# jc-bao/gym-formation

Hardware: AMD Instinct MI355X
Metric: env-steps/sec (higher is better)
Workload: dtype f32

## Files before the change

### gym-formation_amd/csrc/fg_obs_writers.hpp

```cpp
#ifndef FG_OBS_WRITERS_HPP_
#define FG_OBS_WRITERS_HPP_

#include "fg_common.hpp"

namespace fg {

template <class V2> FG_DEV V2 lds_if(bool c, const V2* __restrict__ p, int idx_if_true) {
    V2 t = p[c ? idx_if_true : 0];
    t.x = c ? t.x : 0.0f; t.y = c ? t.y : 0.0f;
    return t;
}

constexpr bool FG_ROWS_MERGED = true;
template <int NC, int NW, int E, int PACE = 0>
FG_DEV void write_obs_rows(const real2* __restrict__ tables0, int env_stride, int w,
                           real2* __restrict__ out_env0, size_t env_units, int El, int parts,
                           int wg_part = 0, int wg_parts = 1, bool pace_on = true) {
    constexpr int N = NC;
    constexpr int WPE = (E >= NW) ? 1 : NW / E;
    constexpr int ESTEP = (E >= NW) ? NW : 1;
    static_assert((E >= NW) ? (E % NW == 0) : (NW % E == 0), "waves and envs must tile");
    const int lane = threadIdx.x & 63;
    const int row0 = (E >= NW) ? 0 : w % WPE;
    constexpr unsigned ROWU = 3u * N;
    for (int ee = (E >= NW) ? w : w / WPE; ee < El; ee += (E >= NW ? ESTEP : E)) {
        const real2* __restrict__ AA = tables0 + (size_t)ee * env_stride;
        real2* __restrict__ out = out_env0 + (size_t)ee * env_units;
        if constexpr (N <= 64) {
            constexpr int RW = 64 / N;
            const int rsub = lane / N, u = lane - rsub * N;
            const bool act = rsub < RW;
            const real2 zero = make_real2(0.f, 0.f);
            const real2 Pm = lds_if(act && u >= 1, AA, u - 1);
            const real2 Pu = lds_if(act && u >= 1, AA, u);
            const int xoff = (u == 0) ? 4 * N : 0;
            constexpr int CS = (2 * N + 63) / 64;
            constexpr int RS = (2 * N <= 64) ? 64 / (2 * N) : 1;
            const int ssub = (2 * N <= 64) ? lane / (2 * N) : 0;
            const int sidx = (2 * N <= 64) ? lane - ssub * 2 * N : lane;
            real2 sv[CS];
#pragma unroll
            for (int c = 0; c < CS; ++c)
                sv[c] = lds_if(ssub < RS && sidx + 64 * c < 2 * N, AA, N + sidx + 64 * c);
#pragma unroll 2
            for (int rb = row0; rb < N; rb += RW * WPE) {
                const int r = rb + rsub * WPE;
                if ((parts & 1) && act && r < N) {
                    const real2 x = AA[xoff + r];
                    const real2 c = (u - 1 >= r) ? Pu : Pm;
                    out[(unsigned)r * ROWU + (unsigned)u] = make_real2(c.x - x.x, c.y - x.y);
                }
#pragma unroll
                for (int k0 = 0; k0 < RW; k0 += RS) {
                    const int rs = rb + (k0 + ssub) * WPE;
                    if ((parts & 2) && ssub < RS && k0 + ssub < RW && rs < N) {
#pragma unroll
                        for (int c = 0; c < CS; ++c)
                            if (sidx + 64 * c < 2 * N) out[(unsigned)rs * ROWU + (unsigned)(N + sidx + 64 * c)] = sv[c];
                    }
                }
            }
        } else if constexpr (FG_ROWS_MERGED && ((3 * N + 63) / 64 < (N + 63) / 64 + (2 * N + 63) / 64)) {
            constexpr int CR = (3 * N + 63) / 64;
            constexpr int C_MIX = N / 64;
            real2 Pm[CR], Pu[CR];
#pragma unroll
            for (int c = 0; c < CR; ++c) {
                const int u = lane + 64 * c;
                if (c <= C_MIX) {
                    const bool dyn = u >= 1 && u < N, stat = u >= N && u < 3 * N;
                    Pm[c] = lds_if(dyn || stat, AA, stat ? u : u - 1);
                    Pu[c] = lds_if(dyn || stat, AA, u);
                } else {
                    Pm[c] = Pu[c] = lds_if(u < 3 * N, AA, u);
                }
            }
            const int nshare = WPE * wg_parts, share = wg_part * WPE + row0;
            const int PER = (N + nshare - 1) / nshare;
            const int r_end = min(N, (share + 1) * PER);
#pragma unroll 2
            for (int r = share * PER; r < r_end; ++r) {
                const real2 xp = AA[r];
                const real2 x0 = AA[(lane == 0 ? 4 * N : 0) + r];
                real2* __restrict__ orow = out + (unsigned)r * ROWU;
#pragma unroll
                for (int c = 0; c < CR; ++c) {
                    const int u = lane + 64 * c;
                    real2 val;
                    if (c < C_MIX || (c == C_MIX && (N % 64) == 0)) {
                        const real2 x = (c == 0) ? x0 : xp;
                        const real2 cc = (u - 1 >= r) ? Pu[c] : Pm[c];
                        val = make_real2(cc.x - x.x, cc.y - x.y);
                    } else if (c == C_MIX) {
                        const bool dyn = u < N;
                        const real2 x = (c == 0) ? x0 : xp;
                        const real2 cc = (u - 1 >= r) ? Pu[c] : Pm[c];
                        val = make_real2(cc.x - (dyn ? x.x : 0.0f), cc.y - (dyn ? x.y : 0.0f));
                    } else {
                        val = Pu[c];
                    }
                    if (u < 3 * N) orow[u] = val;
                }
                if (PACE > 0 && pace_on) __builtin_amdgcn_s_sleep(PACE);
            }
        } else {
            constexpr int CD = (N + 63) / 64, CS = (2 * N + 63) / 64;
            const real2 zero = make_real2(0.f, 0.f);
            real2 Pm[CD], Pu[CD], sv[CS];
#pragma unroll
            for (int c = 0; c < CD; ++c) {
                const int u = lane + 64 * c;
                Pm[c] = lds_if(u >= 1 && u < N, AA, u - 1);
                Pu[c] = lds_if(u >= 1 && u < N, AA, u);
            }
#pragma unroll
            for (int c = 0; c < CS; ++c) sv[c] = lds_if(lane + 64 * c < 2 * N, AA, N + lane + 64 * c);
            const int nshare = WPE * wg_parts, share = wg_part * WPE + row0;
            const int PER = (N + nshare - 1) / nshare;
            const int r_end = min(N, (share + 1) * PER);
#pragma unroll 2
            for (int r = share * PER; r < r_end; ++r) {
                const real2 xp = AA[r];
                const real2 x0 = AA[(lane == 0 ? 4 * N : 0) + r];
                real2* __restrict__ orow = out + (unsigned)r * ROWU;
#pragma unroll
                for (int c = 0; c < CD; ++c) {
                    const int u = lane + 64 * c;
                    const real2 x = (c == 0) ? x0 : xp;
                    const real2 cc = (u - 1 >= r) ? Pu[c] : Pm[c];
                    if ((parts & 1) && u < N) orow[u] = make_real2(cc.x - x.x, cc.y - x.y);
                }
#pragma unroll
                for (int c = 0; c < CS; ++c)
                    if ((parts & 2) && lane + 64 * c < 2 * N) orow[N + lane + 64 * c] = sv[c];
                if (PACE > 0 && pace_on) __builtin_amdgcn_s_sleep(PACE);
            }
        }
    }
}

template <int NC, int RT> constexpr int tile_units() { return (3 * NC * RT + 16 + 2 + 1) & ~1; }

template <int NC, int NW, int E, int RT, bool STREAM>
FG_DEV void write_obs_tiled(const float2* __restrict__ tables0, int env_stride, int w, float2* __restrict__ tiles,
                            float2* __restrict__ out_env0, size_t unit0, size_t env_units, int El) {
    constexpr int N = NC;
    constexpr int WPE = (E >= NW) ? 1 : NW / E;
    static_assert((E >= NW) ? (E % NW == 0) : (NW % E == 0), "waves and envs must tile");
    static_assert(N <= 32 && N % RT == 0, "tiled writer: N <= 32, RT divides N");
    constexpr unsigned ROWU = 3u * N, TU = ROWU * RT;
    constexpr int TILES_ENV = N / RT;
    constexpr int MY_TILES = (TILES_ENV + WPE - 1) / WPE;
    const int lane = threadIdx.x & 63;
    float2* tile0 = tiles + w * 2 * tile_units<NC, RT>();
    constexpr int RW = 64 / N;
    const int rsub = lane / N, u = lane - rsub * N;
    const bool act = rsub < RW;
    const int xoff = (u == 0) ? 4 * N : 0;
    constexpr int RS = 64 / (2 * N);
    const int ssub = lane / (2 * N), sidx = lane - ssub * 2 * N;
    const int e_first = (E >= NW) ? w : w / WPE, e_step = (E >= NW) ? NW : E;
    const int t_first = (E >= NW) ? 0 : w % WPE;
    const int n_env = (El > e_first) ? (El - e_first + e_step - 1) / e_step : 0;
    const int total = n_env * MY_TILES;

    constexpr unsigned ENVU = ROWU * N;
    const unsigned pad = (unsigned)(env_units - ENVU);
    static_assert(!STREAM || (E >= NW && NC >= 16), "streaming form: waves own whole envs, rows of >= 16 units");
    const bool own = STREAM && ((unit0 & 15) == 0) && (pad == 0 || (pad < 16 && (env_units & 15) == 0));
    auto head_units = [&](int ee) -> unsigned {
        return (own && pad == 0) ? (16u - (unsigned)(((size_t)ee * env_units) & 15)) & 15u : 0u;
    };
    auto extra_units = [&](int ee) -> unsigned {
        if (!own) return 0u;
        if (pad) return pad;
        return (ee + 1 < El) ? head_units(ee + 1) : 0u;
    };

    int cur_env = -1;
    const float2* __restrict__ AA = tables0;
    float2 Pm = make_float2(0.f, 0.f), Pu = Pm, sv = Pm;
    auto locate = [&](int t, int& ee, int& r0) {
        const int ie = t / MY_TILES, it = t - ie * MY_TILES;
        ee = e_first + ie * e_step;
        r0 = (t_first + it * WPE) * RT;
    };
    auto compose = [&](int t) {
        int ee, r0; locate(t, ee, r0);
        if (r0 >= N) return;
        if (ee != cur_env) {
            cur_env = ee;
            AA = tables0 + (size_t)ee * env_stride;
            Pm = lds_if(act && u >= 1, AA, u - 1);
            Pu = lds_if(act && u >= 1, AA, u);
            sv = lds_if(ssub < RS, AA, N + sidx);
        }
        const unsigned par = (unsigned)((unit0 + (size_t)ee * env_units + (size_t)r0 * ROWU) & 1);
        float2* img = tile0 + (t & 1) * tile_units<NC, RT>() + par;
#pragma unroll
        for (int rb = 0; rb < RT; rb += RW) {
            const int rl = rb + rsub;
            if (act && rl < RT) {
                const int r = r0 + rl;
                const float2 x = AA[xoff + r];
                const float2 c = (u - 1 >= r) ? Pu : Pm;
                img[(unsigned)rl * ROWU + (unsigned)u] = make_float2(c.x - x.x, c.y - x.y);
            }
        }
#pragma unroll
        for (int rb = 0; rb < RT; rb += RS) {
            const int rl = rb + ssub;
            if (ssub < RS && rl < RT) img[(unsigned)rl * ROWU + (unsigned)(N + sidx)] = sv;
        }
        if (STREAM && r0 + RT == N) {
            const unsigned x = extra_units(ee);
            if ((unsigned)lane < x) {
                float2 val = make_float2(0.f, 0.f);
                if (pad == 0) {
                    static_assert(ROWU >= 16, "the line remainder must stay inside row 0 of the next env");
                    const float2* __restrict__ A1 = tables0 + (size_t)(ee + 1) * env_stride;
                    const float2 a = A1[lane == 0 ? 3 * N : lane], b = A1[0];
                    const bool rel = lane >= 1 && lane < N;
                    val = make_float2(a.x - (rel ? b.x : 0.f), a.y - (rel ? b.y : 0.f));
                }
                img[TU + (unsigned)lane] = val;
            }
        }
    };
    auto stream = [&](int t) {
        int ee, r0; locate(t, ee, r0);
        if (r0 >= N) return;
        const unsigned par = (unsigned)((unit0 + (size_t)ee * env_units + (size_t)r0 * ROWU) & 1);
        const float2* img = tile0 + (t & 1) * tile_units<NC, RT>() + par;
        float2* __restrict__ out = out_env0 + (size_t)ee * env_units + (size_t)r0 * ROWU;
        if constexpr (!STREAM) {
            if (par && lane == 0) out[0] = img[0];
            constexpr unsigned NPMAX = TU >> 1;
            const unsigned npair = (TU - par) >> 1;
            const f32x4* src4 = reinterpret_cast<const f32x4*>(img + par);
            f32x4* __restrict__ dst4 = reinterpret_cast<f32x4*>(out + par);
#pragma unroll
            for (unsigned q0 = 0; q0 < NPMAX; q0 += 64) {
                const unsigned q = q0 + lane;
                if (q < npair) dst4[q] = src4[q];
            }
            if (((TU - par) & 1u) && lane == 63) out[TU - 1] = img[TU - 1];
        } else {
            const unsigned s = (r0 == 0) ? head_units(ee) : 0u;
            const unsigned end = TU + ((r0 + RT == N) ? extra_units(ee) : 0u);
            const unsigned p2 = (par + s) & 1u;
            if (p2 && lane == 0) out[s] = img[s];
            constexpr unsigned NPMAX = (TU + 16) >> 1;
            const unsigned npair = (end - s - p2) >> 1;
            const f32x4* src4 = reinterpret_cast<const f32x4*>(img + s + p2);
            f32x4* __restrict__ dst4 = reinterpret_cast<f32x4*>(out + s + p2);
            constexpr unsigned NFULL = ((TU - 16) >> 1) / 64;
#pragma unroll
            for (unsigned c = 0; c < NFULL; ++c) {
                const f32x4 v = src4[c * 64 + lane];
                asm volatile("s_waitcnt lgkmcnt(0)" ::: "memory");
                dst4[c * 64 + lane] = v;
                asm volatile("" ::: "memory");
                __builtin_amdgcn_s_sleep(1);
            }
#pragma unroll
            for (unsigned q0 = NFULL * 64; q0 < NPMAX; q0 += 64) {
                const unsigned q = q0 + lane;
                if (q < npair) dst4[q] = src4[q];
            }
            if (((end - s - p2) & 1u) && lane == 63) out[end - 1] = img[end - 1];
        }
    };
    if (total > 0) compose(0);
    for (int t = 0; t < total; ++t) {
        if (t + 1 < total) compose(t + 1);
        stream(t);
    }
}

constexpr int FG_WR_GATHER = 64;
template <int NC> constexpr int gather_passes() { return (3 * NC * NC / 2 + 2 + 63) / 64; }
template <int NC> constexpr int gather_lut_units() { return 2 * gather_passes<NC>() * 64 * 2; }

template <int NC>
FG_DEV void build_gather_lut(uint4* __restrict__ lut, int t, int nthreads) {
    constexpr int N = NC, ROWU = 3 * N, TU = ROWU * N, P = gather_passes<NC>() * 64;
    static_assert(N >= 2 && 5 * N < 65536, "gather writer: table offsets are 16-bit, the table's zeros are the 0 operand");
    auto operands = [&](int unit, unsigned& a, unsigned& b) {
        const int r = unit / ROWU, u = unit - r * ROWU;
        if (u == 0) { a = N; b = 4 * N + r; }
        else if (u < N) { a = (u - 1 >= r) ? u : u - 1; b = r; }
        else { a = u; b = N; }
    };
    for (int e = t; e < 2 * P; e += nthreads) {
        const int par = e / P, q = e - par * P;
        const int npair = (TU - par) >> 1;
        const bool tail = ((TU - par) & 1) != 0;
        int unit = -1, kind = 0;
        if (q < npair) { unit = 2 * q + par; kind = 2; }
        else if (par && q == npair) { unit = 0; kind = 1; }
        else if (tail && q == npair + par) { unit = TU - 1; kind = 1; }
        unsigned a0 = N, b0 = N, a1 = N, b1 = N;
        if (kind >= 1) operands(unit, a0, b0);
        if (kind == 2) operands(unit + 1, a1, b1);
        lut[e] = make_uint4(a0 | (b0 << 16), a1 | (b1 << 16), (unsigned)(unit < 0 ? 0 : unit) | ((unsigned)kind << 16), 0u);
    }
}

template <int NC> struct GatherEntries {
    uint32_t ab0[gather_passes<NC>()], ab1[gather_passes<NC>()], dst[gather_passes<NC>()];
    int phase = -1;
};

template <int NC, int NW, int E>
FG_DEV void write_obs_gather(const float2* __restrict__ tables0, int env_stride, int w, const uint4* __restrict__ lut,
                             float2* __restrict__ out_env0, size_t unit0, size_t env_units, int El, GatherEntries<NC>& cache) {
    constexpr int PASSES = gather_passes<NC>(), P = PASSES * 64;
    const int lane = threadIdx.x & 63;
    for (int ee = w; ee < El; ee += NW) {
        const float2* __restrict__ T = tables0 + (size_t)ee * env_stride;
        const size_t first = unit0 + (size_t)ee * env_units;
        float2* __restrict__ out = out_env0 + (size_t)ee * env_units;
        const int phase = (int)(first & 1);
        if (phase != cache.phase) {
            const uint4* __restrict__ L = lut + phase * P + lane;
#pragma unroll
            for (int c = 0; c < PASSES; ++c) {
                const uint4 t = L[c * 64];
                cache.ab0[c] = t.x; cache.ab1[c] = t.y; cache.dst[c] = t.z;
            }
            cache.phase = phase;
        }
        f32x4 val[PASSES];
#pragma unroll
        for (int c = 0; c < PASSES; ++c) {
            const float2 A0 = T[cache.ab0[c] & 0xffffu], B0 = T[cache.ab0[c] >> 16], A1 = T[cache.ab1[c] & 0xffffu], B1 = T[cache.ab1[c] >> 16];
            val[c] = (f32x4){A0.x - B0.x, A0.y - B0.y, A1.x - B1.x, A1.y - B1.y};
        }
#pragma unroll
        for (int c = 0; c < PASSES; ++c) {
            const unsigned kind = cache.dst[c] >> 16, dst = cache.dst[c] & 0xffffu;
            if (kind == 2) *reinterpret_cast<f32x4*>(out + dst) = val[c];
            else if (kind == 1) out[dst] = make_float2(val[c].x, val[c].y);
        }
    }
}

template <int NC, int NW, int E, int CHMAX = 4> struct SpanGather {
    static constexpr int ENVU = 3 * NC * NC, PIECES = E * ENVU / 2, INSTR = (PIECES + 63) / 64, MINE = (INSTR + NW - 1) / NW;
    static_assert((E * ENVU) % 2 == 0, "an even number of units per workgroup span");
    static FG_DEV void setup(uint2* __restrict__ lut, int w, int env_stride) {
        const int lane = threadIdx.x & 63;
        auto operands = [&](int unit) -> uint32_t {
            const int e = unit / ENVU, q = unit - e * ENVU;
            const int r = q / (3 * NC), u = q - r * (3 * NC);
            uint32_t a, b;
            if (u == 0) { a = NC; b = 4 * NC + r; }
            else if (u < NC) { a = (u - 1 >= r) ? u : u - 1; b = r; }
            else { a = u; b = NC; }
            const uint32_t base = (uint32_t)(e * env_stride);
            return (a + base) | ((b + base) << 16);
        };
        for (int t = 0; t < MINE; ++t) {
            const int piece = (w + NW * t) * 64 + lane;
            if (piece < PIECES) lut[piece] = make_uint2(operands(2 * piece), operands(2 * piece + 1));
        }
    }
    static FG_DEV void write(const uint2* __restrict__ lut, const float2* __restrict__ tables0, int w, float2* __restrict__ out) {
        const int lane = threadIdx.x & 63;
        f32x4* const out4 = reinterpret_cast<f32x4*>(out);
        constexpr int CH = MINE < CHMAX ? MINE : CHMAX;
#pragma unroll
        for (int t0 = 0; t0 < MINE; t0 += CH) {
            uint2 ent[CH];
#pragma unroll
            for (int c = 0; c < CH; ++c) {
                const int piece = (w + NW * (t0 + c)) * 64 + lane;
                ent[c] = lut[(t0 + c < MINE && piece < PIECES) ? piece : 0];
            }
            f32x4 val[CH];
#pragma unroll
            for (int c = 0; c < CH; ++c) {
                const float2 A0 = tables0[ent[c].x & 0xffffu], B0 = tables0[ent[c].x >> 16];
                const float2 A1 = tables0[ent[c].y & 0xffffu], B1 = tables0[ent[c].y >> 16];
                val[c] = (f32x4){A0.x - B0.x, A0.y - B0.y, A1.x - B1.x, A1.y - B1.y};
            }
#pragma unroll
            for (int c = 0; c < CH; ++c) {
                const int piece = (w + NW * (t0 + c)) * 64 + lane;
                if (t0 + c < MINE && piece < PIECES) out4[piece] = val[c];
            }
        }
    }
};

constexpr int FG_WR_OBS_F16 = 65, FG_WR_OBS_BF16 = 66;
constexpr bool roll_writer_obs16(int wr) { return wr == FG_WR_OBS_F16 || wr == FG_WR_OBS_BF16; }
template <int NC> constexpr int obs16_rows() { return NC > 9 ? 9 : NC; }
template <int NC, int NW, int E> constexpr int obs16_envs() { return NC <= 9 ? E / NW : 1; }
template <int NC, int NW, int E> constexpr int obs16_tile_words() { return (obs16_envs<NC, NW, E>() * obs16_rows<NC>() * 3 * NC + 3 + 3) & ~3; }

#if !FG_F64
typedef uint32_t u32x4 __attribute__((ext_vector_type(4)));
template <int FMT> FG_DEV uint32_t obs16_pack(float x, float y) {
    if constexpr (FMT == FG_WR_OBS_F16) {
        typedef _Float16 h2 __attribute__((ext_vector_type(2)));
        const h2 v = {(_Float16)x, (_Float16)y};
        return __builtin_bit_cast(uint32_t, v);
    } else {
        typedef __bf16 b2 __attribute__((ext_vector_type(2)));
        const b2 v = {(__bf16)x, (__bf16)y};
        return __builtin_bit_cast(uint32_t, v);
    }
}

template <int NC, int NW, int E, int FMT>
FG_DEV void write_obs16(const float2* __restrict__ tables0, int env_stride, int w, uint32_t* __restrict__ tiles,
                        uint32_t* __restrict__ span, size_t unit0, int El) {
    constexpr int N = NC, RT = obs16_rows<NC>(), ET = obs16_envs<NC, NW, E>(), WORDS = obs16_tile_words<NC, NW, E>();
    static_assert(N <= 32 && N % RT == 0 && E >= NW && E % NW == 0, "16-bit writer: N <= 32, whole rows per tile, whole envs per wave");
    static_assert(ET == 1 || RT == N, "a tile of several envs holds them whole");
    constexpr unsigned ROWU = 3u * N, ENVU = ROWU * N, TU = ROWU * RT;
    constexpr int TILES_ENV = N / RT;
    const int lane = threadIdx.x & 63;
    uint32_t* const tile0 = tiles + w * 2 * WORDS;
    constexpr int RW = 64 / N;
    const int rsub = lane / N, u = lane - rsub * N;
    const bool act = rsub < RW;
    const int xoff = (u == 0) ? 4 * N : 0;
    constexpr int RS = 64 / (2 * N);
    const int ssub = lane / (2 * N), sidx = lane - ssub * 2 * N;
    const int n_env = (El > w) ? (El - w + NW - 1) / NW : 0;
    const int total = ET == 1 ? n_env * TILES_ENV : (w * ET < El ? 1 : 0);
    auto locate = [&](int t, int& ee, int& r0, int& ne) {
        if constexpr (ET == 1) {
            const int ie = t / TILES_ENV;
            ee = w + ie * NW; r0 = (t - ie * TILES_ENV) * RT; ne = 1;
        } else {
            ee = w * ET; r0 = 0; ne = min(ET, El - ee);
        }
    };
    auto compose = [&](int t) {
        int ee, r0, ne; locate(t, ee, r0, ne);
        const unsigned par = (unsigned)((unit0 + (size_t)ee * ENVU + (size_t)r0 * ROWU) & 3);
        uint32_t* img = tile0 + (t & 1) * WORDS + par;
        for (int j = 0; j < ne; ++j, img += TU) {
            const float2* __restrict__ AA = tables0 + (size_t)(ee + j) * env_stride;
            const float2 Pm = lds_if(act && u >= 1, AA, u - 1);
            const float2 Pu = lds_if(act && u >= 1, AA, u);
            const float2 sv = lds_if(ssub < RS, AA, N + sidx);
#pragma unroll
            for (int rb = 0; rb < RT; rb += RW) {
                const int rl = rb + rsub;
                if (act && rl < RT) {
                    const int r = r0 + rl;
                    const float2 x = AA[xoff + r];
                    const float2 c = (u - 1 >= r) ? Pu : Pm;
                    img[(unsigned)rl * ROWU + (unsigned)u] = obs16_pack<FMT>(c.x - x.x, c.y - x.y);
                }
            }
            const uint32_t svp = obs16_pack<FMT>(sv.x, sv.y);
#pragma unroll
            for (int rb = 0; rb < RT; rb += RS) {
                const int rl = rb + ssub;
                if (ssub < RS && rl < RT) img[(unsigned)rl * ROWU + (unsigned)(N + sidx)] = svp;
            }
        }
    };
    auto stream = [&](int t) {
        int ee, r0, ne; locate(t, ee, r0, ne);
        const size_t first = (size_t)ee * ENVU + (size_t)r0 * ROWU;
        const unsigned par = (unsigned)((unit0 + first) & 3);
        const uint32_t* img = tile0 + (t & 1) * WORDS + par;
        uint32_t* __restrict__ out = span + first;
        const unsigned n = (unsigned)ne * TU;
        const unsigned head = (4u - par) & 3u;
        if ((unsigned)lane < head) out[lane] = img[lane];
        const unsigned nq = (n - head) >> 2;
        const u32x4* src4 = reinterpret_cast<const u32x4*>(img + head);
        u32x4* __restrict__ dst4 = reinterpret_cast<u32x4*>(out + head);
        constexpr unsigned NQMAX = ((unsigned)ET * TU) >> 2;
#pragma unroll
        for (unsigned q0 = 0; q0 < NQMAX; q0 += 64) {
            const unsigned q = q0 + lane;
            if (q < nq) dst4[q] = src4[q];
        }
        const unsigned tail = (n - head) & 3u, t0 = head + 4u * nq;
        if ((unsigned)lane < tail) out[t0 + lane] = img[t0 + lane];
    };
    if (total > 0) compose(0);
    for (int t = 0; t < total; ++t) {
        if (t + 1 < total) compose(t + 1);
        stream(t);
    }
}
#endif

}

#endif
```

Baseline: 341.3 million.

## Add compile-time scheduled streaming observation writer interleaving tile build and drain

Adds a specialized observation writer for 27 agents with 9-row tiles and two envs per wave. It unrolls the tile schedule at compile time and interleaves building the next LDS tile with draining the current one through 16-byte global stores. The goal is to hide LDS latency behind global stores and keep output writes aligned. In exchange it adds a lot of geometry-specific code, plus manual waitcnt and sleep instructions that may not suit other configurations.

```diff
diff --git a/gym-formation_amd/csrc/fg_obs_writers.hpp b/gym-formation_amd/csrc/fg_obs_writers.hpp
--- a/gym-formation_amd/csrc/fg_obs_writers.hpp
+++ b/gym-formation_amd/csrc/fg_obs_writers.hpp
@@ -1,6 +1,8 @@
 #ifndef FG_OBS_WRITERS_HPP_
 #define FG_OBS_WRITERS_HPP_
 
+#include <type_traits>
+#include <utility>
 #include "fg_common.hpp"
 
 namespace fg {
@@ -141,9 +143,200 @@
 
 template <int NC, int RT> constexpr int tile_units() { return (3 * NC * RT + 16 + 2 + 1) & ~1; }
 
+struct StreamTile { int env, r0, rows; };
+template <int NC, int NW, int E, int RT> struct StreamSchedule {
+    static constexpr bool enabled = NC == 27 && RT == 9 && E == 2 * NW;
+    static constexpr int EPW = E / NW, PER_ENV = NC / RT, NT = EPW * PER_ENV;
+    static constexpr StreamTile tile(int i) { return {i / PER_ENV, (i % PER_ENV) * RT, RT}; }
+    static constexpr int full_stores(int rows) { return ((3 * NC * rows - 16) >> 1) / 64; }
+};
+template <int... I, class F> FG_DEV void static_for_seq(std::integer_sequence<int, I...>, F&& f) { (f(std::integral_constant<int, I>{}), ...); }
+template <int CNT, class F> FG_DEV void static_for(F&& f) { static_for_seq(std::make_integer_sequence<int, CNT>{}, f); }
+
+template <int NC, int NW, int E, int RT>
+FG_DEV void write_obs_stream(const float2* __restrict__ tables0, int env_stride, int w_lane, float2* __restrict__ tiles,
+                             float2* __restrict__ out_env0, size_t unit0, size_t env_units, int El) {
+    using S = StreamSchedule<NC, NW, E, RT>;
+    static_assert(S::enabled && NC % RT == 0, "scheduled streaming writer: a schedule for this geometry");
+    constexpr int N = NC, EPW = S::EPW, NT = S::NT;
+    constexpr unsigned ROWU = 3u * N, ENVU = ROWU * N;
+    constexpr int RW = 64 / N, RS = 64 / (2 * N);
+    static_assert(RS >= 1 && RW % RS == 0 && ROWU >= 16, "rows of 16 ... 32 agents");
+    const int w = __builtin_amdgcn_readfirstlane(w_lane);
+    const int lane = threadIdx.x & 63;
+    float2* const tile0 = tiles + w * 2 * tile_units<NC, RT>();
+    const int rsub = lane / N, u = lane - rsub * N;
+    const bool act = rsub < RW;
+    const bool cached = act && u >= 1;
+    const int um1_rsub = u - 1 - rsub;
+    const int xoff = (u == 0) ? 4 * N : 0;
+    const int ssub = lane / (2 * N), sidx = lane - ssub * 2 * N;
+    const int n_env = (El > w) ? (El - w + NW - 1) / NW : 0;
+
+    const unsigned pad = (unsigned)(env_units - ENVU);
+    const bool own = ((unit0 & 15) == 0) && (pad == 0 || (pad < 16 && (env_units & 15) == 0));
+    auto head_units = [&](int ee) -> unsigned {
+        return (own && pad == 0) ? (16u - (unsigned)(((size_t)ee * env_units) & 15)) & 15u : 0u;
+    };
+    const float2* AAe[EPW];
+    float2* oute[EPW];
+    unsigned pare[EPW], heade[EPW], extrae[EPW];
+#pragma unroll
+    for (int j = 0; j < EPW; ++j) {
+        const int ee = w + j * NW;
+        const size_t envu = (size_t)ee * env_units;
+        AAe[j] = tables0 + ee * env_stride;
+        oute[j] = out_env0 + envu;
+        pare[j] = (unsigned)((unit0 + envu) & 1);
+        heade[j] = head_units(ee);
+        extrae[j] = !own ? 0u : pad ? pad : (ee + 1 < El) ? head_units(ee + 1) : 0u;
+    }
+
+    float2 Pm = make_float2(0.f, 0.f), Pu = Pm, sv = Pm;
+    float2 px = Pm, pa = Pm, pb = Pm;
+    f32x4 q4 = {0.f, 0.f, 0.f, 0.f};
+    float2 qh = Pm, qt = Pm;
+    auto lds_wait = [] { asm volatile("s_waitcnt lgkmcnt(0)" ::: "memory"); };
+    auto image = [&](auto ti) -> float2* {
+        constexpr int I = decltype(ti)::value;
+        constexpr StreamTile T = S::tile(I);
+        return tile0 + (I & 1) * tile_units<NC, RT>() + (pare[T.env] ^ ((T.r0 * ROWU) & 1u));
+    };
+    auto pass_load = [&](auto ti, auto pi) {
+        constexpr int I = decltype(ti)::value, P = decltype(pi)::value;
+        constexpr StreamTile T = S::tile(I);
+        constexpr int NPASS = (T.rows + RW - 1) / RW;
+        const float2* __restrict__ AA = AAe[T.env];
+        if constexpr (P == 0 && T.r0 == 0) {
+            Pm = AA[cached ? u - 1 : 0];
+            Pu = AA[cached ? u : 0];
+            sv = AA[ssub < RS ? N + sidx : 0];
+        }
+        px = AA[xoff + T.r0 + P * RW + rsub];
+        if constexpr (P == NPASS - 1 && T.r0 + T.rows == N) {
+            if (pad == 0) {
+                const float2* __restrict__ A1 = AA + env_stride;
+                pa = lds_if((unsigned)lane < extrae[T.env], A1, lane == 0 ? 3 * N : lane);
+                pb = lds_if((unsigned)lane < extrae[T.env], A1, 0);
+            }
+        }
+    };
+    auto pass_write = [&](auto ti, auto pi) {
+        constexpr int I = decltype(ti)::value, P = decltype(pi)::value;
+        constexpr StreamTile T = S::tile(I);
+        constexpr int NPASS = (T.rows + RW - 1) / RW;
+        float2* img = image(ti);
+        if constexpr (P == 0 && T.r0 == 0) {
+            Pm.x = cached ? Pm.x : 0.0f; Pm.y = cached ? Pm.y : 0.0f;
+            Pu.x = cached ? Pu.x : 0.0f; Pu.y = cached ? Pu.y : 0.0f;
+            sv.x = ssub < RS ? sv.x : 0.0f; sv.y = ssub < RS ? sv.y : 0.0f;
+        }
+        const int rl = P * RW + rsub;
+        if (act && rl < T.rows) {
+            int d = um1_rsub;
+            asm volatile("" : "+v"(d));
+            const float2 c = (d >= T.r0 + P * RW) ? Pu : Pm;
+            img[(unsigned)rl * ROWU + (unsigned)u] = make_float2(c.x - px.x, c.y - px.y);
+        }
+#pragma unroll
+        for (int k = 0; k < RW; k += RS) {
+            const int rs = P * RW + k + ssub;
+            if (ssub < RS && rs < T.rows) img[(unsigned)rs * ROWU + (unsigned)(N + sidx)] = sv;
+        }
+        if constexpr (P == NPASS - 1 && T.r0 + T.rows == N) {
+            if ((unsigned)lane < extrae[T.env]) {
+                float2 val = make_float2(0.f, 0.f);
+                if (pad == 0) {
+                    const bool rel = lane >= 1 && lane < N;
+                    val = make_float2(pa.x - (rel ? pb.x : 0.f), pa.y - (rel ? pb.y : 0.f));
+                }
+                img[ROWU * T.rows + (unsigned)lane] = val;
+            }
+        }
+    };
+    auto slot = [&](auto ti, auto ci, bool load) {
+        constexpr int I = decltype(ti)::value, C = decltype(ci)::value;
+        constexpr StreamTile T = S::tile(I);
+        constexpr unsigned TU = ROWU * T.rows, NFULL = S::full_stores(T.rows), NPMAX = (TU + 16) >> 1;
+        static_assert(NPMAX - NFULL * 64 <= 64, "one masked store behind the full ones");
+        const unsigned s = (T.r0 == 0) ? heade[T.env] : 0u;
+        const unsigned end = TU + ((T.r0 + T.rows == N) ? extrae[T.env] : 0u);
+        const float2* img = image(ti);
+        float2* __restrict__ out = oute[T.env] + T.r0 * ROWU;
+        const unsigned par = pare[T.env] ^ ((T.r0 * ROWU) & 1u);
+        const unsigned p2 = (par + s) & 1u;
+        const f32x4* src4 = reinterpret_cast<const f32x4*>(img + s + p2);
+        f32x4* __restrict__ dst4 = reinterpret_cast<f32x4*>(out + s + p2);
+        if constexpr (C < NFULL) {
+            if (load) q4 = src4[C * 64 + lane]; else dst4[C * 64 + lane] = q4;
+        } else {
+            const unsigned q = NFULL * 64 + lane, npair = (end - s - p2) >> 1;
+            const bool tail = ((end - s - p2) & 1u) && lane == 63;
+            if (load) {
+                if (q < npair) q4 = src4[q];
+                if (p2 && lane == 0) qh = img[s];
+                if (tail) qt = img[end - 1];
+            } else {
+                if (p2 && lane == 0) out[s] = qh;
+                if (q < npair) dst4[q] = q4;
+                if (tail) out[end - 1] = qt;
+            }
+        }
+    };
+
+    if (n_env > 0) {
+        constexpr StreamTile T = S::tile(0);
+        static_for<(T.rows + RW - 1) / RW>([&](auto pi) {
+            pass_load(std::integral_constant<int, 0>{}, pi);
+            lds_wait();
+            pass_write(std::integral_constant<int, 0>{}, pi);
+        });
+    }
+    static_for<NT>([&](auto ti) {
+        constexpr int I = decltype(ti)::value;
+        constexpr StreamTile T = S::tile(I);
+        constexpr int NFULL = S::full_stores(T.rows), NS = NFULL + 1;
+        if (T.env < n_env) {
+            auto drain = [&] {
+                static_for<NS>([&](auto ci) {
+                    slot(ti, ci, true);
+                    lds_wait();
+                    slot(ti, ci, false);
+                    asm volatile("" ::: "memory");
+                    if constexpr (decltype(ci)::value < NFULL) __builtin_amdgcn_s_sleep(1);
+                });
+            };
+            if constexpr (I + 1 == NT) drain();
+            else {
+                constexpr StreamTile X = S::tile(I + 1);
+                constexpr int NPX = (X.rows + RW - 1) / RW;
+                std::integral_constant<int, I + 1> tn;
+                auto interleaved = [&] {
+                    static_for<(NPX > NS ? NPX : NS)>([&](auto ki) {
+                        constexpr int K = decltype(ki)::value;
+                        if constexpr (K < NPX) pass_load(tn, ki);
+                        if constexpr (K < NS) slot(ti, ki, true);
+                        lds_wait();
+                        if constexpr (K < NS) slot(ti, ki, false);
+                        if constexpr (K < NPX) pass_write(tn, ki);
+                        asm volatile("" ::: "memory");
+                        if constexpr (K >= NPX && K < NFULL) __builtin_amdgcn_s_sleep(1);
+                    });
+                };
+                if constexpr (X.env == T.env) interleaved();
+                else { if (X.env < n_env) interleaved(); else drain(); }
+            }
+        }
+    });
+}
+
 template <int NC, int NW, int E, int RT, bool STREAM>
 FG_DEV void write_obs_tiled(const float2* __restrict__ tables0, int env_stride, int w, float2* __restrict__ tiles,
                             float2* __restrict__ out_env0, size_t unit0, size_t env_units, int El) {
+    if constexpr (STREAM && StreamSchedule<NC, NW, E, RT>::enabled) {
+        write_obs_stream<NC, NW, E, RT>(tables0, env_stride, w, tiles, out_env0, unit0, env_units, El);
+        return;
+    }
     constexpr int N = NC;
     constexpr int WPE = (E >= NW) ? 1 : NW / E;
     static_assert((E >= NW) ? (E % NW == 0) : (NW % E == 0), "waves and envs must tile");
diff --git a/profiles/r06_stream_sched_requests.py b/profiles/r06_stream_sched_requests.py
--- /dev/null
+++ b/profiles/r06_stream_sched_requests.py
@@ -0,0 +1,65 @@
+N, E, NW = 27, 16, 8
+ROWU, ENVU = 3 * N, 3 * N * N
+
+
+def head_units(ee):
+    return (16 - ((ee * ENVU) & 15)) & 15
+
+
+def segments(first_byte, nbytes):
+    return (first_byte + nbytes - 1) // 64 - first_byte // 64 + 1 if nbytes else 0
+
+
+ALIGN = False
+
+
+def tile_stores(ee, r0, rows, El=E):
+    out = ee * ENVU + r0 * ROWU
+    TU = ROWU * rows
+    s = head_units(ee) if r0 == 0 else 0
+    extra = (head_units(ee + 1) if ee + 1 < El else 0) if r0 + rows == N else 0
+    end = TU + extra
+    p2 = (out + s) & 1
+    st = []
+    if p2:
+        st.append(((out + s) * 8, 8))
+    npair = (end - s - p2) >> 1
+    base = (out + s + p2) * 8
+    lead = ((-base) >> 4) & 3 if ALIGN else 0
+    if lead:
+        st.append((base, lead * 16))
+    base += lead * 16
+    nfull = ((TU - 16 - (6 if ALIGN else 0)) >> 1) // 64
+    for c in range(nfull):
+        st.append((base + c * 1024, 1024))
+    rest = npair - lead - nfull * 64
+    assert 0 < rest <= 64
+    st.append((base + nfull * 1024, rest * 16))
+    if (end - s - p2) & 1:
+        st.append(((out + end - 1) * 8, 8))
+    return st
+
+
+def count(first_env_rows, other_rows=(9, 9, 9)):
+    instr = req = nbytes = 0
+    covered = set()
+    for w in range(NW):
+        for j, ee in enumerate(range(w, E, NW)):
+            r0 = 0
+            for rows in (first_env_rows if j == 0 else other_rows):
+                for b, n in tile_stores(ee, r0, rows):
+                    instr += 1; req += segments(b, n); nbytes += n
+                    assert not covered & set(range(b, b + n, 8))
+                    covered |= set(range(b, b + n, 8))
+                r0 += rows
+            assert r0 == N
+    assert nbytes == E * ENVU * 8 and len(covered) == E * ENVU
+    return instr, req
+
+
+if __name__ == "__main__":
+    import sys
+    ALIGN = "--align" in sys.argv
+    print("ideal requests per workgroup-step: %d" % (E * ENVU * 8 // 64))
+    for name, rows in (("9+9+9", (9, 9, 9)), ("ramp 2+7+9+9", (2, 7, 9, 9))) + ((("ramp 4+5+9+9", (4, 5, 9, 9)),) if not ALIGN else ()):
+        print("%-16s store instructions %d, 64-byte requests %d" % ((name,) + count(rows)))
```

Result: faster. 347.3 million (median of 6 runs) (+1.7%).
